# saugns/saugns

Measured on AMD Instinct MI355X. Metric: mono samples/sec/GPU @ N voices (depth-3 FM), higher is better.
Workload: dtype f32 (f64 table interpolation, u32 phase)

## Files before the change

saugns_amd/csrc/k_fast_group_lm.h:

```cpp
		const int j0 = l * T;
		const int t0 = (int)(cg * GF) - (int)H + j0;
		const uint32_t om = ((1u << T) - 1u) & ~((1u << min(max((int)H - j0, 0), T)) - 1u);
		auto prev32 = [&](const uint32_t *x, int k) -> uint32_t { return k > 0 ? x[k - 1] : lane_prev(x[T - 1]); };
		auto prev64 = [&](const double *x, int k) -> double { return k > 0 ? x[k - 1] : lane_prev(x[T - 1]); };
		const bool quads = ((cg * GF - H) & 3u) == 0;
		auto store_row = [&](float *row, const float *x, const bool nt) {
			uint32_t o = om;
			asm volatile("" : "+v"(o));
			if (quads) {
#pragma unroll
				for (int q = 0; q < T / 4; ++q) {
					const uint32_t oq = (o >> (4 * q)) & 15u;
					if (oq == 15u) {
						const fk_f32x4 v4 = {x[4 * q], x[4 * q + 1], x[4 * q + 2], x[4 * q + 3]};
						fk_f32x4 *p = (fk_f32x4 *)(row + t0 + 4 * q);
						if (nt) FK_VSTORE(p, v4); else *p = v4;
					} else if (oq != 0u) {
#pragma unroll
						for (int u = 0; u < 4; ++u)
							if ((oq >> u) & 1u) { if (nt) FK_VSTORE(&row[t0 + 4 * q + u], x[4 * q + u]); else row[t0 + 4 * q + u] = x[4 * q + u]; }
					}
				}
			} else {
#pragma unroll
				for (int k = 0; k < T; ++k)
					if ((o >> k) & 1u) { if (nt) FK_VSTORE(&row[t0 + k], x[k]); else row[t0 + k] = x[k]; }
			}
		};
		uint32_t held_rows = 0;
		bool held_far = false;
		float blk[T];
		for (uint32_t si = 0; si < n_fsteps; ++si) {
			const FastStep f = load_step_uniform(fsteps + si);
			const uint32_t kind = f.kind & 0xff;
			const uint32_t flags = (f.kind >> 8) & 0xff;
			int t0s = t0;
			asm volatile("" : "+v"(t0s));
			{
				const uint32_t o1 = f.out_off + 1u, p1 = f.pm_off + 1u, q1 = f.fpm_off + 1u, a1 = f.amp_off + 1u;
				uint32_t two = 0;
				if (kind == ST_OSC) two = o1 | a1 | (p1 + q1) | (flags & SF_WAVE_ENV);
				else if (kind == ST_LINE) two = o1;
				else if (kind == ST_VOICE) two = o1 | (p1 << 1);
				else if (kind == ST_LERP) two = 2u;
				if (two > 1u) { zero_acc = 1; continue; }
			}
			if (kind == ST_OSC) {
				const uint32_t type = f.type & 0xff;
				const bool layer = (flags & SF_LAYER) != 0;
				const bool to_voice = ((f.kind >> 16) & OX_VOICE) != 0;
				float s[T];
				if (type == OT_WAVE) {
					const bool has_pm = f.pm_off != ~0u, has_fpm = f.fpm_off != ~0u;
					const int p_min = (int)H - (int)(f.kind >> 24) + 1;
					const int nd = min(max(p_min - j0, 0), T);
					const uint32_t dm = ((1u << T) - 1u) & ~((1u << nd) - 1u);
					bool done = false;
					if (FK_COMMON && f.tab >= 0 && !has_fpm && !(f.ramp & 2)) {
						uint32_t ph[T];
						{
							uint32_t acc = f.phase0 + f.inc * (uint32_t)(t0 + 1);
#pragma unroll
							for (int k = 0; k < T; ++k) { ph[k] = acc; acc += f.inc; }
						}
						bool ok = true;
						if (has_pm) {
							float pm[T];
							bool big = false;
#pragma unroll
							for (int k = 0; k < T; ++k) {
								pm[k] = blk[k];
								big |= !(fabsf(pm[k]) < 0x1p20f);
							}
							ok = !__any(big);
#pragma unroll
							for (int k = 0; k < T; ++k) ph[k] += rint32w_p31_small(pm[k]);
						}
						if (ok) {
							const uint32_t ltab = tabs + (uint32_t)f.tab * FkTab<WIDE>::BYTES;
							double Is[T];
#pragma unroll
							for (int k = 0; k < T; ++k) Is[k] = fk_poly(fk_entry<WIDE>(ltab, ph[k]), ph[k]);
							if (FK_CONSTD && !has_pm && f.inc != 0) {
								const double x = (double)div_f32_normal(f.diff_scale, (float)(int32_t)f.inc);
#pragma unroll
								for (int k = 0; k < T; ++k)
									s[k] = (float)((Is[k] - prev64(Is, k)) * x + (double)f.diff_offset);
								done = true;
							} else {
								uint32_t dmin = 0xffffffffu;
#pragma unroll
								for (int k = 0; k < T; ++k) {
									uint32_t pp = prev32(ph, k);
									if (k == 0) asm("" : "+v"(pp));
									const int32_t d = (int32_t)(ph[k] - pp);
									dmin = min(dmin, (uint32_t)d);
									s[k] = wosc_diff(Is[k], prev64(Is, k), d, f.diff_scale, f.diff_offset);
								}
								done = true;
								if (__any(dmin == 0u)) {
									uint32_t hz = 0;
#pragma unroll
									for (int k = 0; k < T; ++k) hz |= ph[k] == prev32(ph, k) ? 1u << k : 0u;
									done = !__any((hz & dm) != 0u);
								}
							}
						}
					}
					if (!done) {
						uint32_t ph[T];
						double Is[T];
						float fv[T];
						{
							uint32_t acc = f.phase0 + f.inc * (uint32_t)(t0 + 1);
#pragma unroll
							for (int k = 0; k < T; ++k) { ph[k] = acc; acc += f.inc; fv[k] = f.fc; }
						}
						if (has_pm && !has_fpm) {
							float pm[T];
							bool big = false;
#pragma unroll
							for (int k = 0; k < T; ++k) {
								pm[k] = blk[k];
								big |= !(fabsf(pm[k]) < 0x1p20f);
							}
							if (!__any(big)) {
#pragma unroll
								for (int k = 0; k < T; ++k) ph[k] += rint32w_p31_small(pm[k]);
							} else {
#pragma unroll
								for (int k = 0; k < T; ++k) ph[k] += rint32w_p31(pm[k]);
							}
						} else if (has_fpm) {
#pragma unroll
							for (int k = 0; k < T; ++k) ph[k] += pm_offset32(false, true, 0.f, blk[k], fv[k]);
						}
						if (f.tab >= 0) {
							const uint32_t ltab = tabs + (uint32_t)f.tab * FkTab<WIDE>::BYTES;
#pragma unroll
							for (int k = 0; k < T; ++k) Is[k] = fk_poly(fk_entry<WIDE>(ltab, ph[k]), ph[k]);
						} else {
							const uint32_t wave = (f.type >> 8) & 0xff;
							const HerpC23 *g23 = P.g_c23 + (size_t)wave * WAVE_LEN;
							const HerpC01 *g01 = P.g_c01 + (size_t)wave * WAVE_LEN;
#pragma unroll
							for (int k = 0; k < T; ++k) {
								const uint32_t ind = ph[k] >> SLEN_BITS;
								Is[k] = herp_poly(g23[ind], g01[ind], ph[k]);
							}
						}
						uint32_t hz = 0;
						if (FK_CONSTD && !has_pm && !has_fpm && f.inc != 0) {
							const double x = (double)div_f32_normal(f.diff_scale, (float)(int32_t)f.inc);
#pragma unroll
							for (int k = 0; k < T; ++k) {
								const double pIs = prev64(Is, k);
								s[k] = (float)((Is[k] - pIs) * x + (double)f.diff_offset);
							}
						} else {
#pragma unroll
							for (int k = 0; k < T; ++k) {
								const uint32_t pph = prev32(ph, k);
								const double pIs = prev64(Is, k);
								const int32_t d = (int32_t)(ph[k] - pph);
								hz |= d == 0 ? 1u << k : 0u;
								s[k] = wosc_diff(Is[k], pIs, d, f.diff_scale, f.diff_offset);
							}
						}
						uint32_t held = hz & dm;
						if (__any(held != 0u)) {
							uint32_t src = dm & ~held;
							auto in_lane = [&]() {
#pragma unroll
								for (int k = 1; k < T; ++k)
									if (((held >> k) & 1u) && ((src >> (k - 1)) & 1u)) { s[k] = s[k - 1]; held &= ~(1u << k); src |= 1u << k; }
							};
							in_lane();
							for (int it = 0; it < 64; ++it) {
								const float sp = __shfl_up(s[T - 1], 1);
								const uint32_t okp = ((uint32_t)__shfl_up((int)src, 1) >> (T - 1)) & 1u;
								bool changed = false;
								if ((held & 1u) && okp && l > 0) { s[0] = sp; held &= ~1u; src |= 1u; changed = true; in_lane(); }
								if (!__any(changed)) break;
							}
							const int jm = min(32, 64 - (int)FAST_REPAIR_SHIFT - (int)H);
							if (held) {
								const int j = j0 + (int)__builtin_ctz(held);
								rep[1] = ((uint32_t)(j % 64 - p_min) << 24) | ((uint32_t)(j / 64) << 20) | (si << 12) | (cg & 0xfff);
							}
							const int nf = jm + p_min - j0;
							const bool far = nf <= 0 ? held != 0u : nf < T ? (held >> nf) != 0u : false;
							if (__any(far)) held_far = true;
							if (jm > 0) {
								unsigned long long run = 0;
#pragma unroll
								for (int L = 0; L * T < 64; ++L)
									run |= (unsigned long long)(uint32_t)__builtin_amdgcn_readlane((int)held, L) << (L * T);
								held_rows |= (uint32_t)((run >> p_min) & ((1ull << jm) - 1ull));
							}
						}
					}
				} else if (type == OT_RASEG) {
					const bool rate2x = (f.type >> 17) & 1;
					const float phase_scale = rate2x ? 0x1p31f * 2 : 0x1p31f;
					const RasParams rp = ras_params((uint32_t)f.tab & 0xff, ((uint32_t)f.tab >> 8) & 0xffff,
							f_bits(f.diff_scale), f_bits(f.diff_offset), ((uint32_t)f.tab >> 24) & 0x7f);
					const unsigned long long inc64 = ((unsigned long long)f.prev_phase << 32) | f.inc;
					const unsigned long long cp0 = (unsigned long long)__double_as_longlong(f.prev_Is);
					const bool has_pm = f.pm_off != ~0u, has_fpm = f.fpm_off != ~0u;
#pragma unroll
					for (int k = 0; k < T; ++k) {
						unsigned long long cp = cp0 + inc64 * (unsigned long long)(long long)(t0s + k);
						if (has_pm || has_fpm)
							cp += (unsigned long long)pm_offset(has_pm, has_fpm,
									has_pm ? blk[k] : 0.f,
									has_fpm ? blk[k] : 0.f, f.fc, phase_scale);
						uint32_t cyc;
						float phf;
						ras_split(cp, cyc, phf);
						s[k] = ras_sample(rp, cyc, phf, true, false);
					}
				} else if (type == OT_NOISE) {
					const uint32_t nz = (f.type >> 8) & 0xff;
					const uint32_t n0 = f.phase0;
#pragma unroll
					for (int k = 0; k < T; ++k) {
						const uint32_t n = n0 + (uint32_t)(t0s + k);
						if (nz == NZ_vi) {
							uint32_t s1 = ranfast32(n);
							uint32_t s0 = ranfast32(n - 1);
							s[k] = fscalei((s1 / 2) - (s0 / 2), 0x1p-31f);
						} else if (nz == NZ_bv) {
							int32_t s1 = noise_bv_term(n);
							int32_t s0 = noise_bv_term(n - 1);
							s[k] = (float)(s1 - s0);
						} else {
							s[k] = noise_stateless(nz, n);
						}
					}
				} else {
#pragma unroll
					for (int k = 0; k < T; ++k) s[k] = f.fc;
				}
				float r[T];
				if (f.amp_off != ~0u) {
#pragma unroll
					for (int k = 0; k < T; ++k) r[k] = blk[k];
				} else if (f.ramp & 1) {
					const FastLine fl = load_line_uniform(flines + si);
#pragma unroll
					for (int k = 0; k < T; ++k) r[k] = fast_line_value(fl, t0s + k);
				} else {
#pragma unroll
					for (int k = 0; k < T; ++k) r[k] = f.ac;
				}
				if (layer) {
#pragma unroll
					for (int k = 0; k < T; ++k) r[k] = mix_combine(blk[k], s[k], r[k], false, true);
				} else {
#pragma unroll
					for (int k = 0; k < T; ++k) r[k] = s[k] * r[k];
				}
				if (to_voice) {
					store_row(vrow, r, true);
				} else {
#pragma unroll
					for (int k = 0; k < T; ++k) blk[k] = r[k];
				}
			} else if (kind == ST_LINE) {
				if (f.ramp) {
					FastLine fl;
					fl.goal_len = 0; fl.hold = f.ac; fl.pad = 0;
					fl.sw = sweep_setup(LN_sah, 0.f, 0.f, 0, 1);
					if (f.ramp & 1) fl = load_line_uniform(flines + si);
#pragma unroll
					for (int k = 0; k < T; ++k) blk[k] = fast_line_value(fl, t0s + k);
				} else {
#pragma unroll
					for (int k = 0; k < T; ++k) blk[k] = f.ac;
				}
			} else if (kind == ST_VOICE) {
				store_row(vrow, blk, true);
				if (prow) {
					float x[T];
#pragma unroll
					for (int k = 0; k < T; ++k) x[k] = f.pan;
					store_row(prow, x, false);
				}
			}
		}
		if (held_rows || held_far) {
			bool noted = false;
			if (P.repair_on && !held_far && (int)(cg * GF) - (int)H >= (int)FAST_REPAIR_SHIFT) {
				uint32_t at = 0;
				if (l == 0) at = atomicAdd(&rep[0], 1u);
				at = uni(at);
				if (at < FAST_MAX_REPAIR) {
					if (l == 0) {
						rep[2 + 2 * at] = cg;
						rep[3 + 2 * at] = held_rows;
						atomicOr(&P.pass_flags[FAST_MAX_LEVELS], 1u);
						atomicOr(&P.work_count[1], 2u);
					}
					noted = true;
				}
			}
			if (!noted) zero_acc = 1;
		}
```

Measured before the change: 246.6 million.

## Software-pipeline table gathers ahead of polynomial eval and differencing

After: 248.3 million, median of 3. No clear change (+0.7%).

```diff
diff --git a/saugns_amd/csrc/k_fast_group_lm.h b/saugns_amd/csrc/k_fast_group_lm.h
--- a/saugns_amd/csrc/k_fast_group_lm.h
+++ b/saugns_amd/csrc/k_fast_group_lm.h
@@ -1,3 +1,11 @@
+#ifndef FK_LM_AHEAD
+#define FK_LM_AHEAD 2
+#endif
+#ifdef FK_LM_SCHED
+#define FK_LM_FENCE() __builtin_amdgcn_sched_barrier(0)
+#else
+#define FK_LM_FENCE() ((void)0)
+#endif
 		const int j0 = l * T;
 		const int t0 = (int)(cg * GF) - (int)H + j0;
 		const uint32_t om = ((1u << T) - 1u) & ~((1u << min(max((int)H - j0, 0), T)) - 1u);
@@ -78,25 +86,53 @@
 						}
 						if (ok) {
 							const uint32_t ltab = tabs + (uint32_t)f.tab * FkTab<WIDE>::BYTES;
+							static_assert(T % 2 == 0 && FK_LM_AHEAD >= 1 && 2 * FK_LM_AHEAD <= T, "pairs of registers");
 							double Is[T];
-#pragma unroll
-							for (int k = 0; k < T; ++k) Is[k] = fk_poly(fk_entry<WIDE>(ltab, ph[k]), ph[k]);
+							FkHerp e[T];
+							auto gather = [&](int n) {
+								e[2 * n] = fk_entry<WIDE>(ltab, ph[2 * n]);
+								e[2 * n + 1] = fk_entry<WIDE>(ltab, ph[2 * n + 1]);
+							};
+							auto pipeline = [&](auto diff) {
+#pragma unroll
+								for (int n = 0; n < FK_LM_AHEAD; ++n) gather(n);
+								asm volatile("" : "+v"(ph[0]), "+v"(ph[1]));
+								FK_LM_FENCE();
+#pragma unroll
+								for (int n = 0; n < T / 2; ++n) {
+									const int k0 = 2 * n, k1 = k0 + 1, ka = 2 * (n + FK_LM_AHEAD);
+									Is[k0] = fk_poly(e[k0], ph[k0]);
+									Is[k1] = fk_poly(e[k1], ph[k1]);
+									if (ka < T) {
+										asm volatile("" : "+v"(Is[k0]), "+v"(Is[k1]), "+v"(ph[ka]), "+v"(ph[ka + 1]));
+										FK_LM_FENCE();
+										gather(n + FK_LM_AHEAD);
+									}
+									asm volatile("" : "+v"(Is[k0]), "+v"(Is[k1]));
+									FK_LM_FENCE();
+									if (n > 0) diff(k0);
+									diff(k1);
+									if (n + 1 < T / 2) {
+										if (n > 0) asm volatile("" : "+v"(s[k0]), "+v"(s[k1]), "+v"(ph[k0 + 2]), "+v"(ph[k1 + 2]));
+										else asm volatile("" : "+v"(s[k1]), "+v"(ph[k0 + 2]), "+v"(ph[k1 + 2]));
+										FK_LM_FENCE();
+									}
+								}
+								diff(0);
+							};
 							if (FK_CONSTD && !has_pm && f.inc != 0) {
 								const double x = (double)div_f32_normal(f.diff_scale, (float)(int32_t)f.inc);
-#pragma unroll
-								for (int k = 0; k < T; ++k)
-									s[k] = (float)((Is[k] - prev64(Is, k)) * x + (double)f.diff_offset);
+								pipeline([&](int k) { s[k] = (float)((Is[k] - prev64(Is, k)) * x + (double)f.diff_offset); });
 								done = true;
 							} else {
 								uint32_t dmin = 0xffffffffu;
-#pragma unroll
-								for (int k = 0; k < T; ++k) {
+								pipeline([&](int k) {
 									uint32_t pp = prev32(ph, k);
 									if (k == 0) asm("" : "+v"(pp));
 									const int32_t d = (int32_t)(ph[k] - pp);
 									dmin = min(dmin, (uint32_t)d);
 									s[k] = wosc_diff(Is[k], prev64(Is, k), d, f.diff_scale, f.diff_offset);
-								}
+								});
 								done = true;
 								if (__any(dmin == 0u)) {
 									uint32_t hz = 0;
```
